# wafgo/rt-depth-map

Hardware: AMD Instinct MI355X
Metric: stereo-pairs/sec, 1280x720 d=64 9x9 SAD (higher is better)
Workload: dtype u8

## Files before the change

### rt-depth-map_amd/csrc/k_basic.hip

```cpp
#include "rtdm_kernels.h"
#include "rtdm_device.h"

#include <cstdlib>

namespace rtdm {

__device__ __forceinline__ int colsum3(unsigned long long a, unsigned long long c, unsigned long long b, int k)
{ return (int)((a >> (8 * k)) & 0xff) + 2 * (int)((c >> (8 * k)) & 0xff) + (int)((b >> (8 * k)) & 0xff); }

__global__ __launch_bounds__(256) void k_prefilter8(Plane8 L, Plane8 R, Plane8W Lp, Plane8W Rp,
                                                    int W, int H, int cap, int n, int nxb)
{
    const int idx = blockIdx.x * 256 + threadIdx.x;
    if (idx >= nxb * H) return;
    const int y = idx / nxb, xb = idx - y * nxb, x0 = xb * 8;
    int f = blockIdx.y;
    const bool right = f >= n;
    if (right) f -= n;
    const Plane8 S = right ? R : L;
    const Plane8W O = right ? Rp : Lp;
    const uint8_t* src = S.base + (size_t)f * S.frame;
    uint8_t* dst = O.base + (size_t)f * O.frame + (size_t)y * O.pitch + x0;
    const int npair = (H >= 2) ? (H & ~1) : 0;
    const int off = cap + PREFILTER_BIAS;
// ... 550 lines not shown
__device__ __forceinline__ uint32_t pk_add(uint32_t a, uint32_t b) { return lr_w(lr_u(a) + lr_u(b)); }
__device__ __forceinline__ uint32_t pk_sub(uint32_t a, uint32_t b) { return lr_w(lr_u(a) - lr_u(b)); }
__device__ __forceinline__ uint32_t pk_subsat_u(uint32_t a, uint32_t b) { return lr_w(__builtin_elementwise_sub_sat(lr_u(a), lr_u(b))); }
__device__ __forceinline__ uint32_t pk_min_u(uint32_t a, uint32_t b) { return lr_w(__builtin_elementwise_min(lr_u(a), lr_u(b))); }
__device__ __forceinline__ uint32_t pk_max_i(uint32_t a, uint32_t b) { return lr_w(__builtin_elementwise_max(lr_s(a), lr_s(b))); }
template <int N> __device__ __forceinline__ uint32_t pk_ashr(uint32_t a) { return lr_w(lr_s(a) >> (short)N); }
template <int N> __device__ __forceinline__ uint32_t pk_shl(uint32_t a) { return lr_w(lr_u(a) << (unsigned short)N); }
__device__ __forceinline__ uint32_t pk_is_zero(uint32_t x)
{ uint32_t r; asm("v_pk_sub_u16 %0, 1, %1 op_sel_hi:[0,1] clamp" : "=v"(r) : "v"(x)); return r; }
__device__ __forceinline__ uint32_t lr_bfi(uint32_t mask, uint32_t a, uint32_t b) { return (a & mask) | (b & ~mask); }
__device__ __forceinline__ void lr_lds_min(uint32_t addr, uint32_t v)
{ __hip_atomic_fetch_min((lr_lds_u32*)(uintptr_t)addr, v, __ATOMIC_RELAXED, __HIP_MEMORY_SCOPE_WORKGROUP); }
__device__ __forceinline__ uint32_t lr_lds_ld(uint32_t addr) { return *(const lr_lds_u32*)(uintptr_t)addr; }
__device__ __forceinline__ void lr_lds_barrier() { asm volatile("s_waitcnt lgkmcnt(0)\n\ts_barrier" ::: "memory"); }
__device__ __forceinline__ unsigned lr_bits8(const uint32_t (&h)[4])
{
    const uint32_t g0 = __builtin_amdgcn_perm(h[1], h[0], 0x06040200u), g1 = __builtin_amdgcn_perm(h[3], h[2], 0x06040200u);
    return __builtin_amdgcn_udot4(g1, 0x80402010u, __builtin_amdgcn_udot4(g0, 0x08040201u, 0u, false), false);
}

template <bool SPK, int NIT>
__global__ __launch_bounds__(512) void k_lrcheck_pk(Plane16W disp, const uint16_t* cost, BMGeom g, int maxDiff16,
                                                    int32_t* label, int32_t* size, uint32_t* runs, int32_t* rowcnt,
                                                    int16_t* headmap, int spkDiff)
{
    extern __shared__ __attribute__((aligned(16))) unsigned char smem[];
    const int W = g.W, INV = g.filtered;
    const int Wp = (W + 7) & ~7;
    const int tid = threadIdx.x, lane = tid & 63, wv = tid >> 6;
    const int half = lane >> 5, hl = lane & 31;
    const int chunk = wv * 32 + hl;
    const size_t per_half = (size_t)Wp * 4 + 16 + (size_t)Wp * 2;
    uint32_t* key = (uint32_t*)(smem + (size_t)half * per_half);
    int16_t* fin = (int16_t*)(key + Wp + 4);
    __shared__ int wsum[2][8];
    const int x0 = chunk * 8;
    const int f = blockIdx.z;
    const int minX1 = max(g.minD + g.D, 0), maxX1 = W + min(g.minD, 0);
    const uint32_t INVpk = (uint32_t)(INV & 0xffff) * 0x00010001u;
    const uint32_t KB = (uint32_t)(uintptr_t)(lr_lds_u32*)key * 0x00010001u;
    const uint32_t TRASH = (uint32_t)W * 0x00010001u, NONE = TRASH + 0x00010001u;
    uint32_t X[4], VOTEM[4], KEEPM[4];
    const auto in_range = [](int x, int lo, int hi) -> uint32_t { return (x >= lo && x < hi) ? 0xffffu : 0u; };
    const uint32_t vlo = (uint32_t)(minX1 & 0xffff) * 0x00010001u, vhl = (uint32_t)max(maxX1 - minX1, 0) * 0x00010001u;
    const uint32_t klo = (uint32_t)(g.vx0 & 0xffff) * 0x00010001u, khl = (uint32_t)max(g.vx1 - g.vx0, 0) * 0x00010001u;
    const uint32_t X0 = (uint32_t)x0 * 0x00010001u + 0x00010000u;
#pragma unroll
    for (int k = 0; k < 4; ++k) {
        X[k] = X0 + (uint32_t)k * 0x00020002u;
        VOTEM[k] = pk_sub(pk_is_zero(pk_subsat_u(vhl, pk_sub(X[k], vlo))), 0x00010001u);
        KEEPM[k] = pk_sub(pk_is_zero(pk_subsat_u(khl, pk_sub(X[k], klo))), 0x00010001u);
    }
    const auto slot_addr = [&](uint32_t idx, uint32_t lim) -> uint32_t { return pk_add(pk_shl<2>(pk_min_u(idx, lim)), KB); };
    const uint32_t Mpk = (uint32_t)maxDiff16 * 0x00010001u;
    const uint32_t Spk = (uint32_t)spkDiff * 0x00010001u, S2pk = Spk + Spk;
    if (chunk == 0) { key[Wp] = ~0u; key[Wp + 1] = ~0u; }
#pragma unroll 1
    for (int it = 0; it < NIT; ++it) {
        const int ypair = 2 * ((int)blockIdx.y * NIT + it);
        if (NIT > 1 && g.vy0 + ypair >= g.vy1) break;
        const int y0 = g.vy0 + ypair, y = y0 + half;
        const bool active = x0 < W && y < g.vy1;
        int16_t* row = disp.base + ((size_t)f * disp.frame_e + (size_t)y0 * disp.pitch_e) + (half ? (uint32_t)disp.pitch_e : 0u);
        [[maybe_unused]] const uint16_t* crow = cost + ((size_t)f * g.H + y0) * g.Ws + (half ? (uint32_t)g.Ws : 0u);
        uint32_t D[4] = {INVpk, INVpk, INVpk, INVpk}, C[4] = {0, 0, 0, 0};
        if (active) {
            const uint4 dq = *(const uint4*)(row + x0), cq = *(const uint4*)(crow + x0);
            D[0] = dq.x; D[1] = dq.y; D[2] = dq.z; D[3] = dq.w; C[0] = cq.x; C[1] = cq.y; C[2] = cq.z; C[3] = cq.w;
            if (x0 + 8 > W) {
#pragma unroll
                for (int k = 0; k < 4; ++k) {
                    const uint32_t m = in_range(x0 + 2 * k, 0, W) | (in_range(x0 + 2 * k + 1, 0, W) << 16);
                    D[k] = lr_bfi(m, D[k], INVpk);
                }
            }
            const uint4 none = make_uint4(~0u, ~0u, ~0u, ~0u);
            ((uint4*)(key + x0))[0] = none; ((uint4*)(key + x0))[1] = none;
        }
        lr_lds_barrier();
        uint32_t V[4], Dx[4];
        if (active) {
#pragma unroll
            for (int k = 0; k < 4; ++k) {
                V[k] = pk_sub(pk_is_zero(D[k] ^ INVpk), 0x00010001u);
                Dx[k] = D[k] ^ 0x80008000u;
                const uint32_t cv = C[k] | ~(V[k] & VOTEM[k]);
                const uint32_t a = slot_addr(pk_sub(X[k], pk_ashr<4>(pk_add(D[k], 0x00080008u))), TRASH);
                lr_lds_min(a & 0xffffu, __builtin_amdgcn_perm(cv, Dx[k], 0x05040100u));
                lr_lds_min(a >> 16, __builtin_amdgcn_perm(cv, Dx[k], 0x07060302u));
            }
        }
        lr_lds_barrier();
        if (active) {
            uint32_t bad0[4], any0 = 0;
#pragma unroll
            for (int k = 0; k < 4; ++k) {
                const uint32_t a = slot_addr(pk_sub(X[k], pk_ashr<4>(D[k])), NONE);
                const uint32_t qe = lr_lds_ld(a & 0xffffu), qo = lr_lds_ld(a >> 16);
                const uint32_t df = pk_sub(__builtin_amdgcn_perm(qo, qe, 0x05040100u), Dx[k]);
                const uint32_t r = pk_sub(Mpk, pk_max_i(df, pk_sub(0u, df)));
                bad0[k] = r & ~__builtin_amdgcn_perm(qo, qe, 0x07060302u) & V[k] & VOTEM[k] & KEEPM[k];
                any0 |= bad0[k];
            }
            uint32_t Dn[4] = {D[0], D[1], D[2], D[3]};
            if (__builtin_amdgcn_ballot_w64((any0 & 0x80008000u) != 0) != 0) {
#pragma unroll
                for (int k = 0; k < 4; ++k) {
                    const uint32_t a = slot_addr(pk_sub(X[k], pk_ashr<4>(pk_add(D[k], 0x000f000fu))), NONE);
                    const uint32_t qe = lr_lds_ld(a & 0xffffu), qo = lr_lds_ld(a >> 16);
                    const uint32_t df = pk_sub(__builtin_amdgcn_perm(qo, qe, 0x05040100u), Dx[k]);
                    const uint32_t r = pk_sub(Mpk, pk_max_i(df, pk_sub(0u, df)));
                    const uint32_t killed = pk_ashr<15>(bad0[k] & r & ~__builtin_amdgcn_perm(qo, qe, 0x07060302u));
                    Dn[k] = lr_bfi(killed, INVpk, D[k]);
                }
            }
            uint32_t chg = 0;
#pragma unroll
            for (int k = 0; k < 4; ++k) {
                Dn[k] = lr_bfi(KEEPM[k], Dn[k], INVpk);
                chg |= Dn[k] ^ D[k];
                D[k] = Dn[k];
            }
            if (chg) *(uint4*)(row + x0) = make_uint4(D[0], D[1], D[2], D[3]);
            if (SPK) *(uint4*)(fin + x0) = make_uint4(D[0], D[1], D[2], D[3]);
        }
        if (!SPK) { if (NIT > 1) { lr_lds_barrier(); continue; } else return; }
        lr_lds_barrier();
        unsigned im = 0, cb = 0;
        if (active) {
            const int left = x0 > 0 ? (int)fin[x0 - 1] : INV, right = x0 + 8 < W ? (int)fin[x0 + 8] : INV;
            uint32_t iz[4], cl[4];
#pragma unroll
            for (int k = 0; k < 4; ++k) {
                iz[k] = pk_is_zero(D[k] ^ INVpk);
                const uint32_t prev = __builtin_amdgcn_alignbit(D[k], k ? D[k - 1] : ((uint32_t)left << 16), 16);
                cl[k] = pk_is_zero(pk_subsat_u(pk_add(pk_sub(D[k], prev), Spk), S2pk));
            }
            im = ~lr_bits8(iz) & 0xffu;
            cb = lr_bits8(cl) & (im & ((im << 1) | (unsigned)(left != INV)));
            cb |= (unsigned)conn((int)(int16_t)(D[3] >> 16), right, INV, spkDiff) << 8;
        }
        const unsigned hm = im & ~cb & 0xffu;
        unsigned lm = im & ~(cb >> 1) & 0xffu;
        const int agg = hm ? ((__builtin_popcount(hm) << 16) | (x0 + (31 - __builtin_clz(hm)) + 1)) : 0;
        int t = agg;
#define RTDM_SCAN(ctrl, rmask) t = OpHead::f(t, __builtin_amdgcn_update_dpp(0, t, ctrl, rmask, 0xf, false))
        RTDM_SCAN(0x111, 0xf); RTDM_SCAN(0x112, 0xf); RTDM_SCAN(0x114, 0xf); RTDM_SCAN(0x118, 0xf);
        RTDM_SCAN(0x142, 0xa);
#undef RTDM_SCAN
        if (hl == 31) wsum[half][wv] = t;
        lr_lds_barrier();
        int run = __builtin_amdgcn_update_dpp(0, t, 0x138, 0xf, 0xf, false);
        if (hl == 0) run = 0;
        for (int q = 0; q < wv; ++q) run = OpHead::f(run, wsum[half][q]);
        if (active) {
            const int base = (f * g.H + y) * g.Ws;
            const int hin = (run & 0xffff) - 1, cin = run >> 16;
            ((uint32_t*)headmap)[(size_t)(f * g.H + y) * (g.Ws >> 3) + chunk] = (uint32_t)cin | (hm << 16);
            while (lm) {
                const int k = __builtin_ctz(lm);
                lm &= lm - 1;
                const unsigned hb = hm & ((2u << k) - 1u);
                const int h = hb ? x0 + (31 - __builtin_clz(hb)) : hin;
                const int node = base + cin + __builtin_popcount(hb) - 1;
                const int len = x0 + k - h + 1;
                label[node] = node;
                size[node] = len;
                runs[node] = (uint32_t)h | ((uint32_t)len << 16);
            }
            if (x0 + 8 >= W) rowcnt[f * g.H + y] = cin + __builtin_popcount(hm);
        }
    }
}

static bool two_ok_for_pk(const BMGeom& g, int md, int spkDiff)
{
    return 2L * g.cap * g.w * g.w < 32768 && md >= 0 && md <= 8192 && spkDiff >= 0 && spkDiff <= 4096 &&
           g.minD >= -1024 && g.minD + g.D <= 1024 && g.W + 2 < 16384;
}

int launch_lrcheck(Plane16W disp, const void* cost, const BMGeom& g, int disp12MaxDiff, int n,
                   hipStream_t stream, int32_t* label, int32_t* size, uint32_t* runs, int32_t* rowcnt,
                   int16_t* headmap, int spkDiff)
{
    const int md = disp12MaxDiff * 16;
    const int nrows = g.vy1 - g.vy0;
    dim3 block(256);
    const bool k32 = g.cost16 && g.W < 65536;
    const size_t kb = k32 ? 4 : 8;
#define RTDM_LR(SPK, CT, KT)                                                                                          \
    hipLaunchKernelGGL((k_lrcheck<SPK, CT, KT, 1>), dim3(1, nrows, n), block, (size_t)g.W * (kb + 2 + (SPK ? 4 : 2)), stream, \
                       disp, (const CT*)cost, g, md, label, size, runs, rowcnt, headmap, spkDiff)
    const int Wp = (g.W + 7) & ~7;
    const bool vec = k32 && (g.Ws & 7) == 0 && g.W <= 4096 && disp.pitch_e >= (size_t)Wp &&
                     (((size_t)disp.base | (disp.pitch_e * 2) | (disp.frame_e * 2) | (size_t)cost | (size_t)headmap) & 15) == 0;
    if (vec) {
        const int chunks = Wp >> 3;
        const auto per_half = [&](int nb) { return (size_t)Wp * 4 + 16 + (size_t)nb * Wp * 2; };
        static const int pairs_raw = env_int("RTDM_LR_PAIRS", 0);
        const int pairs = (pairs_raw == 1 || pairs_raw == 2) ? pairs_raw : ((g.W <= 1024 || (long)n * nrows <= 11520) ? 2 : 1);
        const int waves1 = (chunks + 63) / 64, waves2 = (chunks + 31) / 32;
        const bool two = waves2 <= 8 && nrows >= 2;
        static const int pk_env = env_int("RTDM_LR_PACKED", 1);
        const bool pk_ok = pk_env && two_ok_for_pk(g, md, spkDiff) && 2 * per_half(1) + 1024 < 65536;
        const bool contacts_here = two && label && nrows >= 4 && pairs > 1;
        if (two && pk_ok && !contacts_here) {
            const dim3 vblock((unsigned)(waves2 * 64));
#define RTDM_LRP(SPK) hipLaunchKernelGGL((k_lrcheck_pk<SPK, 1>), dim3(1, (nrows + 1) / 2, n), vblock, 2 * per_half(1), stream, disp, \
                                 (const uint16_t*)cost, g, md, label, size, runs, rowcnt, headmap, spkDiff)
            if (label) RTDM_LRP(true); else RTDM_LRP(false);
#undef RTDM_LRP
            return label ? 1 : 0;
        }
        if (two) {
            const dim3 vblock((unsigned)(waves2 * 64));
            const int nit = (label && nrows >= 4) ? pairs : 1;
#define RTDM_LRV(SPK, NIT) hipLaunchKernelGGL((k_lrcheck_vec<SPK, true, NIT>), dim3(1, (nrows + 2 * NIT - 1) / (2 * NIT), n), vblock, \
                               2 * per_half(NIT > 1 ? 2 : 1), stream, disp, (const uint16_t*)cost, g, md, label, size, runs, rowcnt, headmap, spkDiff)
            if (!label) RTDM_LRV(false, 1);
            else if (nit == 2) RTDM_LRV(true, 2);
            else RTDM_LRV(true, 1);
#undef RTDM_LRV
            return label ? (nit > 1 ? 2 * nit : 1) : 0;
        }
        const dim3 vblock((unsigned)(waves1 * 64));
        const size_t lds = per_half(1);
        if (label) hipLaunchKernelGGL((k_lrcheck_vec<true, false, 1>), dim3(1, nrows, n), vblock, lds, stream, disp, (const uint16_t*)cost, g, md, label, size, runs, rowcnt, headmap, spkDiff);
        else       hipLaunchKernelGGL((k_lrcheck_vec<false, false, 1>), dim3(1, nrows, n), vblock, lds, stream, disp, (const uint16_t*)cost, g, md, label, size, runs, rowcnt, headmap, spkDiff);
        return label ? 1 : 0;
    } else if (label) {
        if (k32) RTDM_LR(true, uint16_t, uint32_t);
        else if (g.cost16) RTDM_LR(true, uint16_t, unsigned long long);
        else RTDM_LR(true, int32_t, unsigned long long);
    } else {
        if (k32) RTDM_LR(false, uint16_t, uint32_t);
        else if (g.cost16) RTDM_LR(false, uint16_t, unsigned long long);
        else RTDM_LR(false, int32_t, unsigned long long);
    }
#undef RTDM_LR
    return 0;
}

__global__ __launch_bounds__(256) void k_spk_init(Plane16W disp, int32_t* label, int32_t* size, uint32_t* runs,
                                                  int32_t* rowcnt, int16_t* headmap, int W, int Ws, int H, int newVal, int maxDiff)
{
    extern __shared__ __attribute__((aligned(16))) unsigned char smem[];
    int* sc = (int*)smem;
    int16_t* d = (int16_t*)(sc + W);
    __shared__ int wsum[4];
    const int y = blockIdx.y, f = blockIdx.z;
    const int16_t* row = disp.base + (size_t)f * disp.frame_e + (size_t)y * disp.pitch_e;
    for (int x = threadIdx.x; x < W; x += 256) d[x] = row[x];
    __syncthreads();
    spk_row_init(d, sc, wsum, W, (f * H + y) * Ws, label, size, runs, rowcnt + (f * H + y), headmap, newVal, maxDiff);
}

__global__ __launch_bounds__(256) void k_spk_merge(Plane16W disp, int32_t* label, const int16_t* headmap, int W, int Ws, int H,
                                                   int y_lo, int npairs, int ystep, int newVal, int maxDiff)
{
    const int nxb = (W + 7) / 8;
    const int idx = blockIdx.x * 256 + threadIdx.x;
    const bool inb = idx < nxb * npairs;
    const int cidx = inb ? idx : 0;
    const int y = y_lo + (cidx / nxb) * ystep, x0 = (cidx % nxb) * 8;
    const int f = blockIdx.y;
    const int16_t* d0 = disp.base + (size_t)f * disp.frame_e + (size_t)y * disp.pitch_e;
    const int16_t* d1 = d0 + disp.pitch_e;
    const int base0 = (f * H + y) * Ws, base1 = base0 + Ws;
    const int16_t* h0 = headmap + base0;
    const int16_t* h1 = headmap + base1;
    Short8 a8, b8, ha8, hb8;
    unsigned cm = 0;
    if (inb) {
        for (int k = 0; k < 8; ++k) { const int x = min(x0 + k, W - 1); a8.v[k] = d0[x]; b8.v[k] = d1[x]; }
#pragma unroll
        for (int k = 0; k < 8; ++k) cm |= (unsigned)((x0 + k < W) && conn(a8.v[k], b8.v[k], newVal, maxDiff)) << k;
    }
    ha8.v[7] = hb8.v[7] = 0;
    if (cm) {
        for (int k = 0; k < 8; ++k) { const int x = min(x0 + k, W - 1); ha8.v[k] = h0[x]; hb8.v[k] = h1[x]; }
    }
    const int packed = (int)(cm >> 7) | ((int)(uint16_t)ha8.v[7] << 1) | ((int)(uint16_t)hb8.v[7] << 17);
    const int fromLeft = __shfl_up(packed, 1);
    if (!cm) return;
    bool pc = false;
    int ph0 = -1, ph1 = -1;
    if (x0 > 0) {
        if ((threadIdx.x & 63) != 0) {
            pc = fromLeft & 1; ph0 = (fromLeft >> 1) & 0xffff; ph1 = (fromLeft >> 17) & 0x7fff;
        } else {
            pc = conn(d0[x0 - 1], d1[x0 - 1], newVal, maxDiff);
            if (pc) { ph0 = h0[x0 - 1]; ph1 = h1[x0 - 1]; }
        }
    }
#pragma unroll
    for (int k = 0; k < 8; ++k) {
        const bool c = (cm >> k) & 1;
        const int ha = ha8.v[k], hb = hb8.v[k];
        if (c && !(pc && ph0 == ha && ph1 == hb)) uf_union(label, base0 + ha, base1 + hb);
        pc = c; ph0 = ha; ph1 = hb;
    }
}

struct MergeRecArgs { int blocks, vy0, nrows, blk, nch; };
template <int RS, bool COMPACT, bool REC = false>
__global__ __launch_bounds__(256) void k_spk_merge_strip(Plane16W disp, int32_t* label, const int16_t* headmap, int W, int Ws, int H,
                                                         int y_lo, int npairs, int newVal, int maxDiff, int32_t* size, int maxSize,
                                                         int ystep, MergeRecArgs ra)
{
    constexpr int QCAP = 1024;
    __shared__ int2 queue[QCAP];
    __shared__ int qn;
    if (threadIdx.x == 0) qn = 0;
    __syncthreads();
    const bool rec_block = REC && (int)blockIdx.x < ra.blocks;
    if (rec_block) {
        const int inblk = ra.blk - 1, nprs = (ra.nrows / ra.blk) * inblk + max(ra.nrows % ra.blk - 1, 0);
        const int ridx = blockIdx.x * 256 + threadIdx.x;
        if (ridx < nprs * ra.nch) {
            const int j = ridx / ra.nch, chunk = ridx - j * ra.nch;
            const int y = ra.vy0 + j + j / inblk + 1;
            const int f = blockIdx.y;
            const uint32_t* heads = (const uint32_t*)headmap;
            const size_t rrow = (size_t)(f * H + y) * (Ws >> 3);
            const uint32_t cb = heads[rrow + chunk];
            unsigned cand = cb >> 24;
            if (cand) {
                const uint32_t ca = heads[rrow - (Ws >> 3) + chunk];
                const unsigned startA = (ca >> 16) & 0xffu, startB = (cb >> 16) & 0xffu;
                const int base = (f * H + y) * Ws;
                while (cand) {
                    const int k = __builtin_ctz(cand);
                    cand &= cand - 1;
                    const unsigned msk = (2u << k) - 1u;
                    const int na = base - Ws + (int)(ca & 0xffffu) + __builtin_popcount(startA & msk) - 1;
                    const int nb = base + (int)(cb & 0xffffu) + __builtin_popcount(startB & msk) - 1;
                    const int slot = atomicAdd(&qn, 1);
                    if (slot < QCAP) queue[slot] = make_int2(na, nb);
                    else uf_union(label, na, nb);
                }
            }
        }
    }
    const int nxb = (W + 7) >> 3;
    const int nstrips = (npairs + RS - 1) / RS;
    const int idx = ((int)blockIdx.x - (REC ? ra.blocks : 0)) * 256 + threadIdx.x;
    const bool inb = !rec_block && idx < nxb * nstrips;
    const int cidx = inb ? idx : 0;
    const int strip = cidx / nxb, x0 = (cidx % nxb) * 8;
    const int y = y_lo + strip * (RS == 1 ? ystep : RS);
    const int nr = inb ? min(RS, npairs - strip * RS) : 0;
    const int f = blockIdx.y;
    const int16_t* d = disp.base + (size_t)f * disp.frame_e + (size_t)y * disp.pitch_e + x0;
    int base = (f * H + y) * Ws;
    const int16_t* h = headmap + base + x0;
    const unsigned colmask = x0 + 8 <= W ? 0xffu : (0xffu >> (x0 + 8 - W));
    Short8 a8, b8, ha8, hb8;
    if (inb) a8 = *(const Short8*)d;
    bool ha_loaded = false;
    const uint32_t* hc = (const uint32_t*)headmap + (size_t)(f * H + y) * (Ws >> 3) + (x0 >> 3);
    uint32_t ca = (COMPACT && inb) ? hc[0] : 0u;
    Short8 rows[COMPACT ? RS : 1];
    uint32_t heads[COMPACT ? RS : 1];
    if constexpr (COMPACT) {
#pragma unroll
        for (int r = 0; r < RS; ++r) {
            const int rr = r < nr ? r + 1 : nr;
            rows[r] = a8; heads[r] = 0u;
            if (inb) { rows[r] = *(const Short8*)(d + (size_t)rr * disp.pitch_e); heads[r] = hc[(size_t)rr * (Ws >> 3)]; }
        }
    }
#pragma unroll
    for (int r = 0; r < RS; ++r) {
        unsigned cm = 0;
        if (r < nr) {
            if constexpr (COMPACT) b8 = rows[r]; else b8 = *(const Short8*)(d + disp.pitch_e);
#pragma unroll
            for (int k = 0; k < 8; ++k) cm |= (unsigned)conn(a8.v[k], b8.v[k], newVal, maxDiff) << k;
            cm &= colmask;
        }
        if constexpr (COMPACT) {
            const uint32_t cb = r < nr ? heads[r] : 0u;
            unsigned leftc = (unsigned)__builtin_amdgcn_update_dpp(0, (int)(cm >> 7), 0x138, 0xf, 0xf, false);
            if ((threadIdx.x & 63) == 0) leftc = (cm && x0 > 0) ? (unsigned)conn(d[-1], d[disp.pitch_e - 1], newVal, maxDiff) : 0u;
            if (x0 == 0) leftc = 0;
            const unsigned startA = (ca >> 16) & 0xffu, startB = (cb >> 16) & 0xffu;
            unsigned cand = cm & ~(((cm << 1) | (leftc & 1u)) & ~startA & ~startB);
            while (cand) {
                const int k = __builtin_ctz(cand);
                cand &= cand - 1;
                const unsigned ma = startA & ((2u << k) - 1u), mb = startB & ((2u << k) - 1u);
                const int ha = (int)(ca & 0xffffu) + __builtin_popcount(ma) - 1;
                const int hb = (int)(cb & 0xffffu) + __builtin_popcount(mb) - 1;
                const int slot = atomicAdd(&qn, 1);
                if (slot < QCAP) queue[slot] = make_int2(base + ha, base + Ws + hb);
                else uf_union(label, base + ha, base + Ws + hb);
            }
            ca = cb;
        } else {
        hb8.v[7] = 0;
        if (cm) {
            if (!ha_loaded) ha8 = *(const Short8*)h;
            hb8 = *(const Short8*)(h + Ws);
        } else ha8.v[7] = 0;
        const int packed = (int)(cm >> 7) | ((int)(uint16_t)ha8.v[7] << 1) | ((int)(uint16_t)hb8.v[7] << 17);
        const int fromLeft = __shfl_up(packed, 1);
        if (cm) {
            bool pc = false;
            int ph0 = -1, ph1 = -1;
            if (x0 > 0) {
                if ((threadIdx.x & 63) != 0) {
                    pc = fromLeft & 1; ph0 = (fromLeft >> 1) & 0xffff; ph1 = (fromLeft >> 17) & 0x7fff;
                } else {
                    pc = conn(d[-1], d[disp.pitch_e - 1], newVal, maxDiff);
                    if (pc) { ph0 = h[-1]; ph1 = h[Ws - 1]; }
                }
            }
#pragma unroll
            for (int k = 0; k < 8; ++k) {
                const bool c = (cm >> k) & 1;
                const int ha = ha8.v[k], hb = hb8.v[k];
                if (c && !(pc && ph0 == ha && ph1 == hb)) {
                    const int slot = atomicAdd(&qn, 1);
                    if (slot < QCAP) queue[slot] = make_int2(base + ha, base + Ws + hb);
                    else uf_union(label, base + ha, base + Ws + hb);
                }
                pc = c; ph0 = ha; ph1 = hb;
            }
        }
        ha8 = hb8; ha_loaded = cm != 0;
        }
        a8 = b8;
        d += disp.pitch_e; h += Ws; base += Ws;
    }
    __syncthreads();
    const int total = min(qn, QCAP);
    for (int i = threadIdx.x; i < total; i += 256) {
        const int a = queue[i].x, b = queue[i].y;
        uf_union_contact(label, size, a, b, maxSize);
    }
}

template <bool DENSE>
__global__ __launch_bounds__(256) void k_spk_count(int32_t* label, int32_t* size, const uint32_t* runs,
                                                   const int32_t* rowcnt, int Ws, int nrows, int maxSize)
{
    const int row = blockIdx.x * 16 + (threadIdx.x >> 4);
    if (row >= nrows) return;
    const int cnt = rowcnt[row], base = row * Ws;
    for (int i = threadIdx.x & 15; i < cnt; i += 16) {
        const uint32_t rn = runs[base + i];
        const int idx = base + (DENSE ? i : (int)(rn & 0xffffu));
        const int root = uf_find(label, idx);
        if (root == idx) continue;
        st_relaxed(&label[idx], root);
        if (ld_relaxed(&size[root]) <= maxSize) atomicAdd(&size[root], ld_relaxed(&size[idx]));
    }
}

template <bool DENSE>
__global__ __launch_bounds__(256) void k_spk_apply(Plane16W disp, const int32_t* label, const int32_t* size,
                                                   const uint32_t* runs, const int32_t* rowcnt, int Ws, int H, int nrows,
                                                   int newVal, int maxSize)
{
    const int row = blockIdx.x * 16 + (threadIdx.x >> 4);
    if (row >= nrows) return;
    const int cnt = rowcnt[row], base = row * Ws;
    const int f = row / H, y = row - f * H;
    int16_t* drow = disp.base + (size_t)f * disp.frame_e + (size_t)y * disp.pitch_e;
    for (int i = threadIdx.x & 15; i < cnt; i += 16) {
        const uint32_t rn = runs[base + i];
        const int x = (int)(rn & 0xffffu), len = (int)(rn >> 16);
        if (len > maxSize) continue;
        int root = base + (DENSE ? i : x);
        for (int p = label[root]; p != root; p = label[root]) root = p;
        if (size[root] <= maxSize)
            for (int k = 0; k < len; ++k) drow[x + k] = (int16_t)newVal;
    }
}

void launch_speckle(Plane16W disp, int32_t* label, int32_t* size, uint32_t* runs, int32_t* rowcnt, int16_t* headmap,
                    int W, int Ws, int H, int n, int newVal, int maxSize, int maxDiff, bool init_done, int premerged_rows,
                    int y_lo, int y_hi, hipStream_t stream, bool compact_heads)
{
    dim3 block(256);
    if (!init_done) {
        y_lo = 0; y_hi = H; premerged_rows = 1;
        hipLaunchKernelGGL(k_spk_init, dim3(1, H, n), block, (size_t)W * 6, stream, disp, label, size, runs, rowcnt, headmap,
                           W, Ws, H, newVal, maxDiff);
    }
    const int step = premerged_rows > 1 ? premerged_rows : 1;
    const int first = y_lo + step - 1;
    const int last = min(y_hi, H) - 2;
    const int npairs = last >= first ? (last - first) / step + 1 : 0;
    MergeRecArgs rec{};
    static const int fuse_rec = env_int("RTDM_MERGE_REC_FUSED", 1);
    if (compact_heads && step > 1) {
        const int nr = min(y_hi, H) - y_lo, inside = (nr / step) * (step - 1) + max(nr % step - 1, 0), nxb = (W + 7) / 8;
        if (inside > 0) {
            if (fuse_rec && npairs > 0) rec = MergeRecArgs{(inside * nxb + 255) / 256, y_lo, nr, step, nxb};
            else hipLaunchKernelGGL(k_spk_merge_rec, dim3((inside * nxb + 255) / 256, n), block, 0, stream, label, (const uint32_t*)headmap, Ws, H, y_lo, nr, step, nxb,
                                    size, maxSize);
        }
    }
    if (npairs > 0) {
        const int nxb = (W + 7) / 8;
        const bool vec = (((size_t)disp.base | (disp.pitch_e * 2) | (disp.frame_e * 2)) & 15) == 0 && (Ws & 7) == 0 &&
                         disp.pitch_e >= (size_t)((W + 7) & ~7);
        if (compact_heads && step > 1) {
            dim3 sgrid((nxb * npairs + 255) / 256 + rec.blocks, n);
            if (rec.blocks) hipLaunchKernelGGL((k_spk_merge_strip<1, true, true>), sgrid, block, 0, stream, disp, label, headmap, W, Ws, H, first, npairs, newVal, maxDiff, size, maxSize, step, rec);
            else hipLaunchKernelGGL((k_spk_merge_strip<1, true>), sgrid, block, 0, stream, disp, label, headmap, W, Ws, H, first, npairs, newVal, maxDiff, size, maxSize, step, MergeRecArgs{});
        } else
        if (compact_heads) {
            int rsc = 4;
            while (rsc > 1 && (long)((nxb * ((npairs + rsc - 1) / rsc) + 255) / 256) * n < 1024) rsc >>= 1;
            dim3 sgrid((nxb * ((npairs + rsc - 1) / rsc) + 255) / 256, n);
            if (rsc == 4)      hipLaunchKernelGGL((k_spk_merge_strip<4, true>), sgrid, block, 0, stream, disp, label, headmap, W, Ws, H, first, npairs, newVal, maxDiff, size, maxSize, 1, MergeRecArgs{});
            else if (rsc == 2) hipLaunchKernelGGL((k_spk_merge_strip<2, true>), sgrid, block, 0, stream, disp, label, headmap, W, Ws, H, first, npairs, newVal, maxDiff, size, maxSize, 1, MergeRecArgs{});
            else               hipLaunchKernelGGL((k_spk_merge_strip<1, true>), sgrid, block, 0, stream, disp, label, headmap, W, Ws, H, first, npairs, newVal, maxDiff, size, maxSize, 1, MergeRecArgs{});
        } else if (vec) {
            dim3 sgrid((nxb * ((npairs + 3) / 4) + 255) / 256, n);
            hipLaunchKernelGGL((k_spk_merge_strip<4, false>), sgrid, block, 0, stream, disp, label, headmap, W, Ws, H, first, npairs, newVal, maxDiff, size, maxSize, 1, MergeRecArgs{});
        } else {
            hipLaunchKernelGGL(k_spk_merge, dim3((nxb * npairs + 255) / 256, n), block, 0, stream, disp, label, headmap, W, Ws, H, first, npairs, step, newVal, maxDiff);
        }
    }
    const int nrows = n * H;
    if (compact_heads) {
        hipLaunchKernelGGL(k_spk_count<true>, dim3((nrows + 15) / 16), block, 0, stream, label, size, runs, rowcnt, Ws, nrows, maxSize);
        hipLaunchKernelGGL(k_spk_apply<true>, dim3((nrows + 15) / 16), block, 0, stream, disp, label, size, runs, rowcnt, Ws, H, nrows, newVal, maxSize);
    } else {
        hipLaunchKernelGGL(k_spk_count<false>, dim3((nrows + 15) / 16), block, 0, stream, label, size, runs, rowcnt, Ws, nrows, maxSize);
        hipLaunchKernelGGL(k_spk_apply<false>, dim3((nrows + 15) / 16), block, 0, stream, disp, label, size, runs, rowcnt, Ws, H, nrows, newVal, maxSize);
    }
}

}
```

Baseline: 72590.

## Skip settled row pairs in speckle merge and pack connectivity tests

In the compact speckle-merge strip kernel, per-row run metadata (runs array) is looked up first to decide which row pairs can still affect labeling. Rows that are empty at this chunk or already belong to oversized runs are marked settled, and their disparity rows are neither loaded nor compared. Remaining comparisons use packed 16-bit saturating subtract/max ops instead of per-element conn calls. This saves global loads and ALU work in exchange for extra metadata gathers and more complex control flow that must exactly match the original connectivity semantics.

```diff
diff --git a/rt-depth-map_amd/csrc/k_basic.hip b/rt-depth-map_amd/csrc/k_basic.hip
--- a/rt-depth-map_amd/csrc/k_basic.hip
+++ b/rt-depth-map_amd/csrc/k_basic.hip
@@ -876,11 +876,31 @@
     }
 }
 
+__device__ __forceinline__ unsigned spk_invalid_pk(const Short8& r, uint32_t INVpk)
+{
+    const uint4 q = __builtin_bit_cast(uint4, r);
+    const uint32_t z[4] = {pk_is_zero(q.x ^ INVpk), pk_is_zero(q.y ^ INVpk), pk_is_zero(q.z ^ INVpk), pk_is_zero(q.w ^ INVpk)};
+    return lr_bits8(z);
+}
+__device__ __forceinline__ unsigned spk_close_pk(const Short8& a, const Short8& b, uint32_t Spk)
+{
+    const uint4 qa = __builtin_bit_cast(uint4, a), qb = __builtin_bit_cast(uint4, b);
+    const uint32_t A[4] = {qa.x, qa.y, qa.z, qa.w}, B[4] = {qb.x, qb.y, qb.z, qb.w};
+    uint32_t c[4];
+#pragma unroll
+    for (int k = 0; k < 4; ++k) {
+        const lr_s2 df = __builtin_elementwise_sub_sat(lr_s(A[k]), lr_s(B[k]));
+        const uint32_t ad = lr_w(__builtin_elementwise_max(df, __builtin_elementwise_sub_sat(lr_s(0u), df)));
+        c[k] = pk_is_zero(pk_subsat_u(ad, Spk));
+    }
+    return lr_bits8(c);
+}
+
 struct MergeRecArgs { int blocks, vy0, nrows, blk, nch; };
 template <int RS, bool COMPACT, bool REC = false>
 __global__ __launch_bounds__(256) void k_spk_merge_strip(Plane16W disp, int32_t* label, const int16_t* headmap, int W, int Ws, int H,
                                                          int y_lo, int npairs, int newVal, int maxDiff, int32_t* size, int maxSize,
-                                                         int ystep, MergeRecArgs ra)
+                                                         int ystep, MergeRecArgs ra, const uint32_t* runs)
 {
     constexpr int QCAP = 1024;
     __shared__ int2 queue[QCAP];
@@ -929,30 +949,62 @@
     int base = (f * H + y) * Ws;
     const int16_t* h = headmap + base + x0;
     const unsigned colmask = x0 + 8 <= W ? 0xffu : (0xffu >> (x0 + 8 - W));
-    Short8 a8, b8, ha8, hb8;
-    if (inb) a8 = *(const Short8*)d;
+    Short8 a8{}, b8{}, ha8, hb8;
+    if (!COMPACT && inb) a8 = *(const Short8*)d;
     bool ha_loaded = false;
     const uint32_t* hc = (const uint32_t*)headmap + (size_t)(f * H + y) * (Ws >> 3) + (x0 >> 3);
     uint32_t ca = (COMPACT && inb) ? hc[0] : 0u;
     Short8 rows[COMPACT ? RS : 1];
     uint32_t heads[COMPACT ? RS : 1];
+    unsigned unsettled = 0, need = 0;
+    const bool pk = COMPACT && maxDiff >= 0 && maxDiff < 32767 && newVal == (int)(int16_t)newVal;
+    const uint32_t INVpk = (uint32_t)(newVal & 0xffff) * 0x00010001u, Spk = (uint32_t)(maxDiff & 0xffff) * 0x00010001u;
+    unsigned inva = 0, invb = 0;
     if constexpr (COMPACT) {
+        const int hp = Ws >> 3;
+#pragma unroll
+        for (int r = 0; r < RS; ++r) heads[r] = inb ? hc[(size_t)(r < nr ? r + 1 : nr) * hp] : 0u;
+        uint32_t look[RS + 1];
+#pragma unroll
+        for (int j = 0; j <= RS; ++j) {
+            const uint32_t rec = j ? heads[j - 1] : ca;
+            look[j] = runs[(size_t)base + (size_t)(j <= nr ? j : nr) * Ws + (max((int)(rec & 0xffffu), 1) - 1)];
+        }
+        unsigned empty = 0, lng = 0;
+#pragma unroll
+        for (int j = 0; j <= RS; ++j) {
+            const uint32_t rec = j ? heads[j - 1] : ca;
+            const int cnt = (int)(rec & 0xffffu), rx = (int)(look[j] & 0xffffu), rlen = (int)(look[j] >> 16);
+            const bool nostart = (rec & 0xff0000u) == 0u;
+            const bool e = nostart && (cnt == 0 || rx + rlen <= x0);
+            empty |= (unsigned)e << j;
+            lng |= (unsigned)(nostart && !e && rlen > maxSize) << j;
+        }
+        unsettled = ~(empty | (empty >> 1) | (lng & (lng >> 1))) & ((1u << nr) - 1u);
+        need = unsettled | (unsettled << 1);
+        if (need & 1u) a8 = *(const Short8*)d;
 #pragma unroll
         for (int r = 0; r < RS; ++r) {
-            const int rr = r < nr ? r + 1 : nr;
-            rows[r] = a8; heads[r] = 0u;
-            if (inb) { rows[r] = *(const Short8*)(d + (size_t)rr * disp.pitch_e); heads[r] = hc[(size_t)rr * (Ws >> 3)]; }
-        }
+            rows[r] = Short8{};
+            if ((need >> (r + 1)) & 1u) rows[r] = *(const Short8*)(d + (size_t)(r + 1) * disp.pitch_e);
+        }
+        if (pk && (need & 1u)) inva = spk_invalid_pk(a8, INVpk);
     }
 #pragma unroll
     for (int r = 0; r < RS; ++r) {
         unsigned cm = 0;
-        if (r < nr) {
-            if constexpr (COMPACT) b8 = rows[r]; else b8 = *(const Short8*)(d + disp.pitch_e);
-#pragma unroll
-            for (int k = 0; k < 8; ++k) cm |= (unsigned)conn(a8.v[k], b8.v[k], newVal, maxDiff) << k;
+        if constexpr (COMPACT) b8 = rows[r];
+        if constexpr (COMPACT) if (pk && ((need >> (r + 1)) & 1u)) invb = spk_invalid_pk(b8, INVpk);
+        if (COMPACT ? ((unsettled >> r) & 1u) != 0 : r < nr) {
+            if constexpr (!COMPACT) b8 = *(const Short8*)(d + disp.pitch_e);
+            if (COMPACT && pk) cm = spk_close_pk(a8, b8, Spk) & ~(inva | invb);
+            else {
+#pragma unroll
+                for (int k = 0; k < 8; ++k) cm |= (unsigned)conn(a8.v[k], b8.v[k], newVal, maxDiff) << k;
+            }
             cm &= colmask;
         }
+        inva = invb;
         if constexpr (COMPACT) {
             const uint32_t cb = r < nr ? heads[r] : 0u;
             unsigned leftc = (unsigned)__builtin_amdgcn_update_dpp(0, (int)(cm >> 7), 0x138, 0xf, 0xf, false);
@@ -1083,19 +1135,19 @@
                          disp.pitch_e >= (size_t)((W + 7) & ~7);
         if (compact_heads && step > 1) {
             dim3 sgrid((nxb * npairs + 255) / 256 + rec.blocks, n);
-            if (rec.blocks) hipLaunchKernelGGL((k_spk_merge_strip<1, true, true>), sgrid, block, 0, stream, disp, label, headmap, W, Ws, H, first, npairs, newVal, maxDiff, size, maxSize, step, rec);
-            else hipLaunchKernelGGL((k_spk_merge_strip<1, true>), sgrid, block, 0, stream, disp, label, headmap, W, Ws, H, first, npairs, newVal, maxDiff, size, maxSize, step, MergeRecArgs{});
+            if (rec.blocks) hipLaunchKernelGGL((k_spk_merge_strip<1, true, true>), sgrid, block, 0, stream, disp, label, headmap, W, Ws, H, first, npairs, newVal, maxDiff, size, maxSize, step, rec, runs);
+            else hipLaunchKernelGGL((k_spk_merge_strip<1, true>), sgrid, block, 0, stream, disp, label, headmap, W, Ws, H, first, npairs, newVal, maxDiff, size, maxSize, step, MergeRecArgs{}, runs);
         } else
         if (compact_heads) {
             int rsc = 4;
             while (rsc > 1 && (long)((nxb * ((npairs + rsc - 1) / rsc) + 255) / 256) * n < 1024) rsc >>= 1;
             dim3 sgrid((nxb * ((npairs + rsc - 1) / rsc) + 255) / 256, n);
-            if (rsc == 4)      hipLaunchKernelGGL((k_spk_merge_strip<4, true>), sgrid, block, 0, stream, disp, label, headmap, W, Ws, H, first, npairs, newVal, maxDiff, size, maxSize, 1, MergeRecArgs{});
-            else if (rsc == 2) hipLaunchKernelGGL((k_spk_merge_strip<2, true>), sgrid, block, 0, stream, disp, label, headmap, W, Ws, H, first, npairs, newVal, maxDiff, size, maxSize, 1, MergeRecArgs{});
-            else               hipLaunchKernelGGL((k_spk_merge_strip<1, true>), sgrid, block, 0, stream, disp, label, headmap, W, Ws, H, first, npairs, newVal, maxDiff, size, maxSize, 1, MergeRecArgs{});
+            if (rsc == 4)      hipLaunchKernelGGL((k_spk_merge_strip<4, true>), sgrid, block, 0, stream, disp, label, headmap, W, Ws, H, first, npairs, newVal, maxDiff, size, maxSize, 1, MergeRecArgs{}, runs);
+            else if (rsc == 2) hipLaunchKernelGGL((k_spk_merge_strip<2, true>), sgrid, block, 0, stream, disp, label, headmap, W, Ws, H, first, npairs, newVal, maxDiff, size, maxSize, 1, MergeRecArgs{}, runs);
+            else               hipLaunchKernelGGL((k_spk_merge_strip<1, true>), sgrid, block, 0, stream, disp, label, headmap, W, Ws, H, first, npairs, newVal, maxDiff, size, maxSize, 1, MergeRecArgs{}, runs);
         } else if (vec) {
             dim3 sgrid((nxb * ((npairs + 3) / 4) + 255) / 256, n);
-            hipLaunchKernelGGL((k_spk_merge_strip<4, false>), sgrid, block, 0, stream, disp, label, headmap, W, Ws, H, first, npairs, newVal, maxDiff, size, maxSize, 1, MergeRecArgs{});
+            hipLaunchKernelGGL((k_spk_merge_strip<4, false>), sgrid, block, 0, stream, disp, label, headmap, W, Ws, H, first, npairs, newVal, maxDiff, size, maxSize, 1, MergeRecArgs{}, runs);
         } else {
             hipLaunchKernelGGL(k_spk_merge, dim3((nxb * npairs + 255) / 256, n), block, 0, stream, disp, label, headmap, W, Ws, H, first, npairs, step, newVal, maxDiff);
         }
```

Result: faster. 73480, median of 6 (+1.2%).
